# Griffan/FASTQuick

Hardware: AMD Instinct MI355X
Metric: paired_150bp_reads_aligned_per_sec (higher is better)
Workload: dtype u32

## Files before the change

fastquick_amd/csrc/fq_device.hip:

```cpp
#include <hip/hip_runtime.h>
#include <hip/hip_ext.h>

#include <algorithm>
#include <condition_variable>
#include <atomic>
#include <cstdio>
#include <cstdlib>
#include <cstring>
#include <mutex>
#include <string>
#include <unordered_map>
#include <vector>
#include <sys/mman.h>
#include <sys/syscall.h>
#include <unistd.h>

#include "fq_backend.h"

namespace fqdev {

struct Pending { int kid; hipEvent_t a, b; };
struct State {
  int device = 0;
  hipStream_t stream = nullptr;
// ... 368 lines not shown
  uint32_t *cursor;
  const uint32_t *split;
  uint32_t n_work;
  int pref, seg, n_seg;
  __device__ uint64_t operator()(uint32_t n) const {
    const uint32_t sp = split ? *split : n_work;
    const uint32_t blk_start[2] = {0u, sp}, blk_len[2] = {sp, n_work - sp};
    for (int t = 0; t < 2; ++t) {
      const int b = t == 0 ? pref : 1 - pref;
      uint32_t lo, hi;
      fq_seg_range(blk_len[b], seg, n_seg, &lo, &hi);
      const uint32_t len = hi - lo;
      if (len == 0) continue;
      if (__hip_atomic_load(&cursor[b], __ATOMIC_RELAXED, __HIP_MEMORY_SCOPE_AGENT) >= len) continue;
      const uint32_t base = atomicAdd(&cursor[b], n);
      if (base < len) return (uint64_t)(blk_start[b] + lo + base) | (uint64_t)(blk_start[b] + hi) << 32;
    }
    return 0;
  }
};
#define FQ_LANE_FETCH(a) FqQueueFetch2{(a).queue, (a).split, (uint32_t)(a).n_work, (int)((blockIdx.x & 7u) >> 2), (a).seg, (a).n_seg}
__global__ void __launch_bounds__(64) FQ_GAP_OCC k_gap_persist_lds(FqGapArgs a) {
  uint16_t *heads = (uint16_t *)fq_dyn_lds;
  FqGapStoreLds st = {heads + threadIdx.x, 64, (uint32_t *)(heads + 64 * a.o.n_buckets) + threadIdx.x};
  fq_gap_lanes<false>(a, st, FQ_LANE_FETCH(a), (int)(blockIdx.x * 64 + threadIdx.x));
}
__global__ void __launch_bounds__(64) FQ_NOGAP_OCC k_gap_nogap_lds(FqGapArgs a) {
  uint16_t *heads = (uint16_t *)fq_dyn_lds;
  FqGapStoreLds st = {heads + threadIdx.x, 64, (uint32_t *)(heads + 64 * a.o.n_buckets) + threadIdx.x};
  fq_gap_lanes<true>(a, st, FQ_LANE_FETCH(a), (int)(blockIdx.x * 64 + threadIdx.x));
}
__global__ void __launch_bounds__(64) FQ_GAP_OCC k_gap_persist_stock(FqGapArgs a) {
  uint16_t *heads = (uint16_t *)fq_dyn_lds;
  FqGapStoreLds st = {heads + threadIdx.x, 64, (uint32_t *)(heads + 64 * a.o.n_buckets) + threadIdx.x};
  fq_gap_lanes<false, FqOptsStock>(a, st, FQ_LANE_FETCH(a), (int)(blockIdx.x * 64 + threadIdx.x));
}
__global__ void __launch_bounds__(64) FQ_NOGAP_OCC k_gap_nogap_stock(FqGapArgs a) {
  uint16_t *heads = (uint16_t *)fq_dyn_lds;
  FqGapStoreLds st = {heads + threadIdx.x, 64, (uint32_t *)(heads + 64 * a.o.n_buckets) + threadIdx.x};
  fq_gap_lanes<true, FqOptsStock>(a, st, FQ_LANE_FETCH(a), (int)(blockIdx.x * 64 + threadIdx.x));
}
__global__ void __launch_bounds__(64) k_gap_persist(FqGapArgs a) {
  FqGapStoreGlobal st = {nullptr, {}};
  fq_gap_lanes<false>(a, st, FQ_LANE_FETCH(a), (int)(blockIdx.x * 64 + threadIdx.x));
}
__global__ void __launch_bounds__(64) k_gap_coop(FqGapArgs a) {
  __shared__ uint32_t heads[2 * FQ_MAX_BUCKETS];
  fq_gap_coop_wave(a, heads, FqQueueFetch{a.queue, a.n_work}, (int)blockIdx.x);
}
__global__ void __launch_bounds__(256) k_sa(FqSaArgs a) {
  const uint64_t q = (uint64_t)blockIdx.x * blockDim.x + threadIdx.x;
  if (q < a.n_rows) fq_sa_thread(a, q);
}
template <bool PACKED>
__device__ int fq_global_align_wave(const uint8_t *s1, int len1, const uint8_t *s2, int len2, int band, int gap_end,
                                    int *RM, int *RI, int *RD, uint8_t *trace, uint8_t *ops, int *n_ops, int *fi, int *fj);
__device__ __forceinline__ int fq_wave_incl_max(int x, int lane) {
#pragma unroll
  for (int d = 1; d < 64; d <<= 1) { const int y = __shfl_up(x, d, 64); if (lane >= d) x = x > y ? x : y; }
  return x;
}
__device__ void fq_sw_reverse_wave(const uint8_t *ref, const uint8_t *qry, int score_f, int end_i, int end_j, int *H, int *E, int *start_i_out, int *start_j_out, int *score_r_out) {
  const int lane = threadIdx.x;
  const int q = FQ_GAP_O, rr = FQ_GAP_E, qr = q + rr;
  const int kNeg = -(1 << 29);
  for (int i = lane; i <= end_i; i += 64) { H[i] = 0; E[i] = 0; }
  __syncthreads();
  int score_r = fq_sm_maq(ref[end_i - 1], qry[end_j - 1]);
  int start_i = end_i, start_j = end_j;
  if (lane == 0) { H[end_i] = qr + score_r; E[end_i] = 0; }
  __syncthreads();
  int start = end_i - 1, end = end_i - 3;
  if (end <= 0) end = 0;
  bool stop = false;
  for (int j = end_j - 1; j != 0; --j) {
    const int c2 = qry[j - 1];
    const int n = start - end;
    int carry_b = kNeg, carry_m = score_r;
    int d_in = 0, s_in = 0, e_in = 0;
    if (lane < n) { const int i = start - lane; d_in = H[i + 1]; s_in = H[i]; e_in = E[i + 1]; }
    for (int g0 = 0; g0 < n; g0 += 64) {
      const int g = g0 + lane, i = start - g;
      const bool act = g < n;
      int d_nx = 0, s_nx = 0, e_nx = 0;
      if (g + 64 < n) { const int i2 = i - 64; d_nx = H[i2 + 1]; s_nx = H[i2]; e_nx = E[i2 + 1]; }
      int e = e_in - rr > s_in - qr ? e_in - rr : s_in - qr;
      if (e < 0) e = 0;
      int a0 = act ? d_in + fq_sm_maq(ref[i - 1], c2) : 0;
      if (a0 < 0) a0 = 0;
      if (a0 < e) a0 = e;
      const int b = act ? a0 - q + g * rr : kNeg;
      const int bi = fq_wave_incl_max(b, lane);
      int bx = __shfl_up(bi, 1, 64);
      if (lane == 0) bx = kNeg;
      if (bx < carry_b) bx = carry_b;
      const int fpos = bx - g * rr;
      const int h = a0 > fpos ? a0 : fpos;
      const int b_last = __shfl(bi, 63, 64);
      if (carry_b < b_last) carry_b = b_last;
      const int mi = fq_wave_incl_max(act ? h : kNeg, lane);
      int mx = __shfl_up(mi, 1, 64);
      if (lane == 0) mx = kNeg;
      if (mx < carry_m) mx = carry_m;
      const bool improve = act && h > mx;
      const unsigned long long stops = __ballot(improve && h - qr == score_f);
      if (stops) {
        const int ls = __ffsll((long long)stops) - 1;
// ... 51 lines not shown
    for (int d = 32; d >= 1; d >>= 1) nn += __shfl_xor(nn, d, 64);
    if ((float)nn / len >= 0.25f || len - nn < 20) ok = false;
    const int64_t avail = l_pac - T.beg;
    len1 = (int)(avail < (int64_t)T.reglen ? avail : (int64_t)T.reglen);
    if (len1 < 0) len1 = 0;
    for (int k = lane; k < len1; k += 64) ref[k] = (uint8_t)fq_pac_base(a.ix.pac, T.beg + k);
    for (int k = lane; k <= len1 + 1; k += 64) { Hb[k] = 0; Eb[k] = 0; }
  }
  __syncthreads();
  if (!ok) { if (lane == 0) a.out[t] = O; return; }
  const int len2 = len;
  int best_h = 0, best_i = 0, best_j = 0;
  for (int j0 = 0; j0 < len2; j0 += 64) {
    const int j = j0 + lane + 1;
    const bool active = j <= len2;
    const int c2 = active ? qry[j - 1] : 4;
    const int nrows = len2 - j0 < 64 ? len2 - j0 : 64;
    int last_h = 0, f = 0, diag = 0, out_h = 0, out_e = 0;
    const int steps = len1 + nrows - 1;
    for (int st = 1; st <= steps; ++st) {
      int up_h = __shfl_up(out_h, 1, 64), up_e = __shfl_up(out_e, 1, 64);
      const int i = st - lane;
      const bool in = active && i >= 1 && i <= len1;
      if (lane == 0 && in) { up_h = Hb[i]; up_e = Eb[i]; }
      if (in) {
        int e_out;
        const int h = fq_sw_cell(diag, up_h, up_e, fq_sm_maq(ref[i - 1], c2), last_h, f, e_out);
        diag = up_h;
        out_h = h; out_e = e_out;
        if (best_h < h) { best_h = h; best_i = i; best_j = j; }
        if (lane == nrows - 1) { Hb[i] = h; Eb[i] = e_out; }
      }
    }
    __syncthreads();
  }
#pragma unroll
  for (int d = 32; d >= 1; d >>= 1) {
    const int oh = __shfl_xor(best_h, d, 64), oi = __shfl_xor(best_i, d, 64), oj = __shfl_xor(best_j, d, 64);
    if (oh > best_h || (oh == best_h && oh > 0 && oj < best_j)) { best_h = oh; best_i = oi; best_j = oj; }
  }
  if (best_h < 1) { if (lane == 0) a.out[t] = O; return; }
  FqDpScratch S = fq_dp_carve(a.scratch + (size_t)t * a.scratch_stride, RL, QL);
  uint8_t *ops = qry + ((QL + 16) & ~15);
  uint8_t *trace = a.trace_in_lds ? ops + ((RL + QL + 16) & ~15) : S.trace;
  int start_i = 0, start_j = 0, score_r = 0;
  if (a.serial_reverse) {
    if (lane == 0) fq_sw_reverse(ref, qry, best_h, best_i, best_j, Hb, Eb, &start_i, &start_j, &score_r);
    start_i = __shfl(start_i, 0); start_j = __shfl(start_j, 0); score_r = __shfl(score_r, 0);
  } else fq_sw_reverse_wave(ref, qry, best_h, best_i, best_j, Hb, Eb, &start_i, &start_j, &score_r);
  __syncthreads();
  int n_ops = 0, fi = 0, fj = 0, score_g;
  const int jmax = (best_i - start_i > best_j - start_j ? best_i - start_i : best_j - start_j) + 1;
  for (int b = FQ_BAND;; b <<= 1) {
    score_g = fq_global_align_wave<false>(ref + start_i - 1, best_i - start_i + 1, qry + start_j - 1, best_j - start_j + 1, b, -1, rM, rI, rD, trace, ops, &n_ops, &fi, &fj);
    if (score_g == score_r || best_h == score_g) break;
    if (b > jmax) break;
  }
  if (lane == 0) {
    if (!(score_r > score_g && best_h > score_g))
      fq_sw_post(T, ref, qry, len, best_j, start_i, start_j, fi, fj, ops, n_ops, a.cigar + (size_t)t * (size_t)a.cig_cap, a.cig_cap, O);
    a.out[t] = O;
  }
}

__global__ void __launch_bounds__(64) k_refine_lds(FqRefineArgs a) {
  const int t = blockIdx.x * 64 + threadIdx.x;
  int *base = (int *)fq_dyn_lds;
  const int W = a.RL + 1;
  FqRowsPlanar R = {base + threadIdx.x, base + (size_t)W * 64 + threadIdx.x, base + (size_t)2 * W * 64 + threadIdx.x, 64};
  if (t < a.n_task) fq_refine_task(a, t, R);
}
template <bool PACKED>
__device__ __forceinline__ uint8_t fq_trace_get(const uint8_t *trace, int W, int j, int i) {
  if (!PACKED) return trace[(size_t)j * W + i];
  return (uint8_t)((trace[(size_t)j * ((W + 1) >> 1) + (i >> 1)] >> (4 * (i & 1))) & 15);
}
template <bool PACKED>
__device__ int fq_global_align_wave(const uint8_t *s1, int len1, const uint8_t *s2, int len2, int band, int gap_end,
                                    int *RM, int *RI, int *RD, uint8_t *trace, uint8_t *ops, int *n_ops, int *fi, int *fj) {
  const int lane = threadIdx.x;
  if (len1 == 0 || len2 == 0) { *n_ops = 0; return 0; }
  int b1, b2;
  if (len1 > len2) { b1 = len1 - len2 + band; b2 = band; } else { b1 = band; b2 = len2 - len1 + band; }
  if (b1 > len1) b1 = len1;
  if (b2 > len2) b2 = len2;
  const int W = len1 + 1;
  const int end_ext = gap_end >= 0 ? gap_end : FQ_GAP_E;
  if (lane == 0) {
    uint8_t fm;
    int lM = 0, lD = FQ_NEG_INF;
    RM[0] = 0; RI[0] = RD[0] = FQ_NEG_INF;
    for (int i = 1; i < b1; ++i) {
      const int d = fq_pick_gap(lM, lD, end_ext, fm);
      if (PACKED) { uint8_t *b = trace + (i >> 1); *b = (uint8_t)((i & 1) ? ((*b & 15) | ((fm ? 0 : 8) << 4)) : (fm ? 0 : 8)); }
      else trace[i] = (uint8_t)(fm ? 0 : 8);
      RM[i] = RI[i] = FQ_NEG_INF; RD[i] = d;
      lM = FQ_NEG_INF; lD = d;
    }
  }
  __syncthreads();
  const int p1_end = b2 < len2 ? b2 : len2 - 1;
  for (int j0 = 1; j0 <= len2; j0 += 64) {
    const int j = j0 + lane;
    const bool row_on = j <= len2;
    int phase;
    if (j <= p1_end) phase = 1;
    else if (j == p1_end + 1 && j == len2 && b2 != len2 - 1) phase = 5;
    else if (j <= len2 - b2 + 1) phase = 2;
    else if (j < len2) phase = 3;
    else phase = 4;
    const bool p15 = phase == 1 || phase == 5, endD = phase == 5 || phase == 4;
    const int c0 = p15 ? 0 : j - b2;
    const int hi = !row_on ? -1 : p15 ? ((j + b1 <= len1 + 1) ? j + b1 - 1 : len1) : (phase == 2 ? j + b1 - 1 : len1);
    const int c2 = row_on ? s2[j - 1] : 0;
    const bool keeps_row = row_on && (lane == 63 || j == len2);
    uint8_t *tr = trace + (size_t)j * (size_t)(PACKED ? (W + 1) >> 1 : W);
    uint32_t half = 0;
    const int n_rows = len2 - j0 + 1 < 64 ? len2 - j0 + 1 : 64;
    const int t0 = __shfl(c0, 0), t1 = len1 + n_rows - 1;
    int oM = 0, oI = 0, oD = 0;
    FqCell diag, left;
    diag.M = diag.I = diag.D = 0; left = diag;
    for (int t = t0; t <= t1; ++t) {
      const int i = t - lane;
      FqCell up;
      up.M = __shfl_up(oM, 1); up.I = __shfl_up(oI, 1); up.D = __shfl_up(oD, 1);
      if (lane == 0) { const int ii = i < 0 ? 0 : (i > len1 ? len1 : i); up.M = RM[ii]; up.I = RI[ii]; up.D = RD[ii]; }
      if (row_on && i >= c0 && i <= hi) {
        FqCell c;
        uint8_t fm;
        if (i == c0) {
          c.M = c.I = c.D = FQ_NEG_INF;
          uint8_t tb0 = 0;
          if (p15) { c.I = fq_pick_gap(up.M, up.I, end_ext, fm); tb0 = (uint8_t)(fm ? 0 : 4); }
          if (!PACKED) { if (p15) tr[0] = tb0; }
          else if (i & 1) tr[i >> 1] = (uint8_t)(tb0 << 4);
          else { half = tb0; tr[i >> 1] = tb0; }
        } else {
          uint8_t tM, tb;
          c.M = fq_pick_M(diag, fq_sm_maq(s1[i - 1], c2), tM);
          tb = tM;
          if (i != hi) { c.I = fq_pick_gap(up.M, up.I, FQ_GAP_E, fm); tb |= (uint8_t)(fm ? 0 : 4); }
          else if (p15) {
            if (j + b1 - 1 > len1) { c.I = fq_pick_gap(up.M, up.I, end_ext, fm); tb |= (uint8_t)(fm ? 0 : 4); }
            else c.I = FQ_NEG_INF;
          } else if (phase == 2) c.I = FQ_NEG_INF;
          else { c.I = fq_pick_gap(up.M, up.I, end_ext, fm); tb |= (uint8_t)(fm ? 0 : 4); }
          c.D = fq_pick_gap(left.M, left.D, endD ? end_ext : FQ_GAP_E, fm);
          tb |= (uint8_t)(fm ? 0 : 8);
          if (!PACKED) tr[i] = tb;
          else if (i & 1) tr[i >> 1] = (uint8_t)(half | (uint32_t)tb << 4);
          else { half = tb; tr[i >> 1] = tb; }
        }
        diag = up; left = c;
        oM = c.M; oI = c.I; oD = c.D;
        if (keeps_row) { RM[i] = c.M; RI[i] = c.I; RD[i] = c.D; }
      }
    }
    __syncthreads();
  }
  int mx = 0, n = 0, li = 0, lj = 0;
  if (lane == 0) {
    int i = len1, j = len2;
    mx = RM[len1];
    uint8_t tb = fq_trace_get<PACKED>(trace, W, j, i);
    int type = tb & 3, ctype = FQ_OP_M;
    if (RI[len1] > mx) { mx = RI[len1]; type = (tb & 4) ? FQ_OP_I : FQ_OP_M; ctype = FQ_OP_I; }
    if (RD[len1] > mx) { mx = RD[len1]; type = (tb & 8) ? FQ_OP_D : FQ_OP_M; ctype = FQ_OP_D; }
    li = i; lj = j;
    ops[n++] = (uint8_t)ctype;
    do {
      if (ctype == FQ_OP_M) { --i; --j; } else if (ctype == FQ_OP_I) --j; else --i;
      ctype = type;
      tb = fq_trace_get<PACKED>(trace, W, j, i);
      type = type == FQ_OP_M ? (tb & 3) : type == FQ_OP_I ? ((tb & 4) ? FQ_OP_I : FQ_OP_M) : ((tb & 8) ? FQ_OP_D : FQ_OP_M);
      if (i || j) { ops[n++] = (uint8_t)ctype; li = i; lj = j; }
    } while (i || j);
  }
  __syncthreads();
  *n_ops = __shfl(n, 0); *fi = __shfl(li, 0); *fj = __shfl(lj, 0);
  return __shfl(mx, 0);
}
__global__ void __launch_bounds__(64) k_refine_wave(FqRefineArgs a) {
  const int t = blockIdx.x, lane = threadIdx.x;
  const int RL = a.RL, QL = a.QL;
  int *RM = (int *)fq_dyn_lds, *RI = RM + (RL + 1), *RD = RI + (RL + 1);
  uint8_t *ref = (uint8_t *)(RD + (RL + 1));
  uint8_t *qry = ref + ((RL + 16) & ~15);
  uint8_t *ops = qry + ((QL + 16) & ~15);
  uint8_t *trace = ops + ((RL + QL + 16) & ~15);
  const FqRefTask T = a.task[t];
  const int len = a.len_trim[T.read];
  const uint8_t *row = a.seq + (size_t)T.read * (size_t)a.stride;
  const int64_t l_pac = a.ix.l_pac;
  for (int k = lane; k < len; k += 64) qry[k] = (uint8_t)(T.strand ? fq_comp(fq_nt4(row[len - 1 - k])) : fq_nt4(row[k]));
  int64_t pos = (int64_t)T.pos > l_pac ? (int64_t)(int32_t)T.pos : (int64_t)T.pos;
  const int aext = T.ext < 0 ? -T.ext : T.ext, ref_len = len + aext;
  int64_t k0, k1;
  if (T.ext > 0) { k0 = pos; k1 = pos + ref_len < l_pac ? pos + ref_len : l_pac; }
  else { const int64_t x = pos + len; k0 = x - ref_len > 0 ? x - ref_len : 0; k1 = x < l_pac ? x : l_pac; }
  const int l = k1 > k0 ? (int)(k1 - k0) : 0;
  for (int k = lane; k < l; k += 64) ref[k] = (uint8_t)fq_pac_base(a.ix.pac, k0 + k);
  __syncthreads();
  int n_ops = 0, fi, fj;
  fq_global_align_wave<true>(ref, l, qry, len, FQ_BAND, FQ_GAP_END, RM, RI, RD, trace, ops, &n_ops, &fi, &fj);
  if (lane != 0) return;
  uint16_t *cg = a.cigar + (size_t)t * (size_t)a.cig_cap;
  int n = fq_ops_to_cigar(ops, n_ops, cg, a.cig_cap);
  FqRefOut O;
  if (n <= 0) { O.pos = T.pos; O.n_cigar = 0; a.out[t] = O; return; }
  if (T.ext < 0) {
    int d = 0;
    for (int k = 0; k < n; ++k) { const int op = cg[k] >> 14, ln = cg[k] & 0x3fff; if (op == FQ_OP_D) d -= ln; else if (op == FQ_OP_I) d += ln; }
    pos += d;
  }
  if ((cg[0] >> 14) == FQ_OP_D) { pos += cg[0] & 0x3fff; for (int k = 0; k < n - 1; ++k) cg[k] = cg[k + 1]; --n; }
  if ((cg[n - 1] >> 14) == FQ_OP_D) --n;
  if ((cg[n - 1] >> 14) == FQ_OP_I) cg[n - 1] = (uint16_t)(FQ_OP_S << 14 | (cg[n - 1] & 0x3fff));
  if ((cg[0] >> 14) == FQ_OP_I) cg[0] = (uint16_t)(FQ_OP_S << 14 | (cg[0] & 0x3fff));
  O.pos = (uint32_t)pos; O.n_cigar = n;
  a.out[t] = O;
}
__global__ void __launch_bounds__(64) k_refine(FqRefineArgs a) {
  const int t = blockIdx.x * blockDim.x + threadIdx.x;
  if (t < a.n_task) fq_refine_thread(a, t);
}
__global__ void __launch_bounds__(256) k_pack_aln(const FqAln *aln, const uint32_t *n_aln, const uint64_t *off, uint32_t cap, uint32_t n_work, FqAln *packed) {
  const uint32_t w = blockIdx.x * blockDim.x + threadIdx.x;
  if (w >= n_work) return;
  const uint32_t n = n_aln[w];
  const uint64_t o = off[w];
  for (uint32_t j = 0; j < n; ++j) packed[o + j] = aln[(size_t)w * cap + j];
}

__device__ __forceinline__ uint32_t block_excl_scan(uint32_t v, uint32_t *total) {
  __shared__ uint32_t wsum[4];
  const int lane = threadIdx.x & 63, wid = threadIdx.x >> 6;
  uint32_t x = v;
#pragma unroll
  for (int d = 1; d < 64; d <<= 1) {
    const uint32_t y = __shfl_up(x, d, 64);
    if (lane >= d) x += y;
  }
  if (lane == 63) wsum[wid] = x;
  __syncthreads();
  uint32_t base = 0, tot = 0;
#pragma unroll
  for (int k = 0; k < 4; ++k) { if (k < wid) base += wsum[k]; tot += wsum[k]; }
  __syncthreads();
  *total = tot;
  return base + x - v;
}

__global__ void __launch_bounds__(256) k_scan_a(const uint32_t *in, uint32_t n, uint64_t *blk_tot) {
  const uint32_t i = blockIdx.x * 256 + threadIdx.x;
  uint32_t tot;
  (void)block_excl_scan(i < n ? in[i] : 0u, &tot);
  if (threadIdx.x == 0) blk_tot[blockIdx.x] = tot;
}
__global__ void __launch_bounds__(256) k_scan_b(uint64_t *blk_tot, uint32_t nb) {
  __shared__ uint64_t carry;
  if (threadIdx.x == 0) carry = 0;
  __syncthreads();
  for (uint32_t base = 0; base < nb; base += 256) {
    const uint32_t i = base + threadIdx.x;
    const uint64_t v = i < nb ? blk_tot[i] : 0;
    const int lane = threadIdx.x & 63, wid = threadIdx.x >> 6;
    __shared__ uint64_t ws[4];
    uint64_t x = v;
#pragma unroll
    for (int d = 1; d < 64; d <<= 1) {
      const uint64_t y = __shfl_up(x, d, 64);
      if (lane >= d) x += y;
// ... 563 lines not shown
  }
  FQ_HIP(hipGetLastError());
  return 0;
}
int launch_pack_aln(const FqAln *aln, const uint32_t *n_aln, const uint64_t *off, uint32_t cap, uint32_t n_work, FqAln *packed) {
  FQ_PRE();
  if (!n_work) return 0;
  hipLaunchKernelGGL(k_pack_aln, dim3(nblk(n_work, 256)), dim3(256), 0, g_stream, aln, n_aln, off, cap, n_work, packed);
  FQ_HIP(hipGetLastError());
  return 0;
}
int launch_sa(const FqSaArgs &a) {
  FQ_PRE();
  if (!a.n_rows) return 0;
  hipEvent_t e0, e1;
  kernel_events(FQ_K_SA_KERNEL, &e0, &e1);
  hipExtLaunchKernelGGL(k_sa, dim3(nblk(a.n_rows, 256)), dim3(256), 0, g_stream, e0, e1, 0, a);
  FQ_HIP(hipGetLastError());
  return 0;
}
static const size_t kLdsBudget = 150 * 1024;
int launch_sw(const FqSwArgs &a) {
  FQ_PRE();
  if (a.n_task <= 0) return 0;
  size_t lds = (size_t)(2 * (a.RL + 2) + 3 * (a.RL + 1)) * 4 + ((a.RL + 16) & ~15) + ((a.QL + 16) & ~15) + ((a.RL + a.QL + 16) & ~15);
  if (lds > kLdsBudget) { g_err = "SW window too large for LDS (" + std::to_string(a.RL) + " bases)"; return -5; }
  FqSwArgs b = a;
  const size_t trace_bytes = (size_t)(a.RL + 1) * (a.QL + 1) + 16;
  b.trace_in_lds = (lds + trace_bytes <= kLdsBudget && a.n_task <= 256) ? 1 : 0;
  b.serial_reverse = g_cur->tune.sw_serial_reverse;
  if (b.trace_in_lds) lds += trace_bytes;
  hipEvent_t e0, e1;
  kernel_events(FQ_K_SW_KERNEL, &e0, &e1);
  hipExtLaunchKernelGGL(k_sw_wave, dim3((unsigned)a.n_task), dim3(64), lds, g_stream, e0, e1, 0, b);
  FQ_HIP(hipGetLastError());
  return 0;
}
__global__ void __launch_bounds__(64) k_sw_thread(FqSwArgs a) {
  const int t = blockIdx.x * blockDim.x + threadIdx.x;
  if (t < a.n_task) fq_sw_thread(a, t);
}
int launch_sw_serial(const FqSwArgs &a) {
  FQ_PRE();
  if (a.n_task <= 0) return 0;
  hipEvent_t e0, e1;
  kernel_events(FQ_K_SW_KERNEL, &e0, &e1);
  hipExtLaunchKernelGGL(k_sw_thread, dim3(nblk((uint64_t)a.n_task, 64)), dim3(64), 0, g_stream, e0, e1, 0, a);
  FQ_HIP(hipGetLastError());
  return 0;
}
int launch_refine(const FqRefineArgs &a) {
  FQ_PRE();
  if (a.n_task <= 0) return 0;
  const size_t wave_lds = (size_t)3 * (a.RL + 1) * 4 + ((a.RL + 16) & ~15) + ((a.QL + 16) & ~15) + ((a.RL + a.QL + 16) & ~15) + (size_t)((a.RL + 2) >> 1) * (a.QL + 1) + 16;
  const bool no_wave = g_cur->tune.refine_lanes != 0;
  hipEvent_t e0, e1;
  kernel_events(FQ_K_REFINE_KERNEL, &e0, &e1);
  if (wave_lds <= 64 * 1024 && !no_wave) {
    hipExtLaunchKernelGGL(k_refine_wave, dim3((unsigned)a.n_task), dim3(64), wave_lds, g_stream, e0, e1, 0, a);
    FQ_HIP(hipGetLastError());
    return 0;
  }
  const size_t lds = (size_t)3 * (a.RL + 1) * 64 * 4;
  if (lds <= kLdsBudget) {
    hipExtLaunchKernelGGL(k_refine_lds, dim3(nblk((uint64_t)a.n_task, 64)), dim3(64), lds, g_stream, e0, e1, 0, a);
  } else {
    hipExtLaunchKernelGGL(k_refine, dim3(nblk((uint64_t)a.n_task, 64)), dim3(64), 0, g_stream, e0, e1, 0, a);
  }
  FQ_HIP(hipGetLastError());
  return 0;
}

#define FQ_REC_KERNEL(name, body)                                                    \
  __global__ void __launch_bounds__(256) name(FqRecArgs a, int n) {                  \
    const int i = blockIdx.x * blockDim.x + threadIdx.x;                             \
    if (i < n) body(a, i);                                                           \
  }
FQ_REC_KERNEL(k_rec_init, fq_rec_init_thread)
FQ_REC_KERNEL(k_rec_nocc, fq_rec_nocc_thread)
FQ_REC_KERNEL(k_enum_plan, fq_enum_plan_thread)
FQ_REC_KERNEL(k_enum_fill, fq_enum_fill_thread)
FQ_REC_KERNEL(k_main_hit, fq_main_hit_thread)
FQ_REC_KERNEL(k_compact_idx, fq_compact_thread)
FQ_REC_KERNEL(k_pair_rec, fq_pair_rec_thread)
FQ_REC_KERNEL(k_pair_gather, fq_pair_gather_thread)
FQ_REC_KERNEL(k_pair_scatter, fq_pair_scatter_thread)
FQ_REC_KERNEL(k_xa_count, fq_xa_count_thread)
FQ_REC_KERNEL(k_xa_fill, fq_xa_fill_thread)
FQ_REC_KERNEL(k_sw_plan, fq_sw_plan_thread)
FQ_REC_KERNEL(k_sw_fill, fq_sw_fill_thread)
FQ_REC_KERNEL(k_rec_gather, fq_rec_gather_thread)
FQ_REC_KERNEL(k_rec_scatter, fq_rec_scatter_thread)
FQ_REC_KERNEL(k_ref_count, fq_ref_count_thread)
FQ_REC_KERNEL(k_ref_fill, fq_ref_fill_thread)
FQ_REC_KERNEL(k_ref_apply, fq_ref_apply_thread)
FQ_REC_KERNEL(k_md_rec, fq_md_rec_thread)
FQ_REC_KERNEL(k_md_mask, fq_md_mask_piece)
FQ_REC_KERNEL(k_flat_count, fq_flat_count_thread)
FQ_REC_KERNEL(k_flat_fill, fq_flat_fill_thread)
int launch_rec(int op, const FqRecArgs &a, int64_t n) {
  FQ_PRE();
  if (n <= 0) return 0;
  if (n > 0x7fffffff) { g_err = "record stage: more than 2^31 items"; return -5; }
  typedef void (*Kern)(FqRecArgs, int);
  static const Kern kerns[FQ_ROP_COUNT] = {k_rec_init, k_rec_nocc, k_enum_plan, k_enum_fill, k_main_hit, k_compact_idx, k_pair_rec, k_pair_gather, k_pair_scatter,
                                           k_xa_count, k_xa_fill, k_sw_plan, k_sw_fill, k_rec_gather, k_rec_scatter, k_ref_count, k_ref_fill, k_ref_apply,
                                           k_md_rec, k_md_mask, k_flat_count, k_flat_fill};
// ... 172 lines not shown
```

fastquick_amd/csrc/fq_kernels.h:

```cpp
#pragma once
#include "fq_common.h"

#define FQ_LAMBDA_INLINE __attribute__((always_inline))
#if defined(__HIP_DEVICE_COMPILE__)
#define FQ_POPC64(x) __popcll(x)
#define FQ_POPC32(x) __popc(x)
#define FQ_CTZ32(x) (__ffs((int)(x)) - 1)
#define FQ_C_STRIPE_OFF ((size_t)(blockIdx.x & (FQ_C_STRIPES - 1)) * FQ_C_STRIDE)
#define FQ_ATOMIC_ADD64(p, v) atomicAdd((unsigned long long *)(p) + FQ_C_STRIPE_OFF, (unsigned long long)(v))
#define FQ_ATOMIC_MAX64(p, v) atomicMax((unsigned long long *)(p) + FQ_C_STRIPE_OFF, (unsigned long long)(v))
#define FQ_LOAD_RELAXED(p) __hip_atomic_load((p), __ATOMIC_RELAXED, __HIP_MEMORY_SCOPE_AGENT)
#define FQ_ATOMIC_MAX32(p, v) do { const int fq_v_ = (int)(v); if (fq_v_ > FQ_LOAD_RELAXED((const int *)(p))) atomicMax((int *)(p), fq_v_); } while (0)
#define FQ_WAVE_COUNT(p, pred)                                                                                      \
  do {                                                                                                              \
    const unsigned long long m_ = __ballot((pred) ? 1 : 0);                                                         \
    if ((pred) && __lane_id() == (unsigned)(__ffsll((long long)m_) - 1)) atomicAdd((unsigned long long *)(p) + FQ_C_STRIPE_OFF, (unsigned long long)__popcll(m_)); \
  } while (0)
#else
#define FQ_WAVE_COUNT(p, pred) do { if (pred) *(p) += 1; } while (0)
#define FQ_LOAD_RELAXED(p) (*(p))
#define FQ_ATOMIC_MAX32(p, v) (*(p) = *(p) > (int32_t)(v) ? *(p) : (int32_t)(v))
#define FQ_ATOMIC_MAX64(p, v) (*(p) = *(p) > (uint64_t)(v) ? *(p) : (uint64_t)(v))
#define FQ_POPC64(x) __builtin_popcountll(x)
#define FQ_POPC32(x) __builtin_popcount(x)
// ... 1836 lines not shown
      diag = R.get(j - b2);
      left.M = left.I = left.D = FQ_NEG_INF;
      R.set(j - b2, left);
    }
    for (int i = lo; i <= hi; ++i) {
      const FqCell up = R.get(i);
      FqCell c;
      uint8_t tM, tb;
      c.M = fq_pick_M(diag, fq_sm_maq(s1[i - 1], c2), tM);
      tb = tM;
      if (i != hi) { c.I = fq_pick_gap(up.M, up.I, FQ_GAP_E, fm); tb |= (uint8_t)(fm ? 0 : 4); }
      else if (phase == 1 || phase == 5) {
        if (j + b1 - 1 > len1) { c.I = fq_pick_gap(up.M, up.I, end_ext, fm); tb |= (uint8_t)(fm ? 0 : 4); }
        else c.I = FQ_NEG_INF;
      } else if (phase == 2) c.I = FQ_NEG_INF;
      else { c.I = fq_pick_gap(up.M, up.I, end_ext, fm); tb |= (uint8_t)(fm ? 0 : 4); }
      c.D = fq_pick_gap(left.M, left.D, endD ? end_ext : FQ_GAP_E, fm);
      tb |= (uint8_t)(fm ? 0 : 8);
      tr[i] = tb;
      R.set(i, c);
      diag = up;
      left = c;
    }
  }
  const FqCell last = R.get(len1);
  int i = len1, j = len2, mx = last.M;
  uint8_t tb = trace[(size_t)j * W + i];
  int type = tb & 3, ctype = FQ_OP_M;
  if (last.I > mx) { mx = last.I; type = (tb & 4) ? FQ_OP_I : FQ_OP_M; ctype = FQ_OP_I; }
  if (last.D > mx) { mx = last.D; type = (tb & 8) ? FQ_OP_D : FQ_OP_M; ctype = FQ_OP_D; }
  int n = 0, li = i, lj = j;
  ops[n++] = (uint8_t)ctype;
  do {
    if (ctype == FQ_OP_M) { --i; --j; } else if (ctype == FQ_OP_I) --j; else --i;
    ctype = type;
    tb = trace[(size_t)j * W + i];
    type = type == FQ_OP_M ? (tb & 3) : type == FQ_OP_I ? ((tb & 4) ? FQ_OP_I : FQ_OP_M) : ((tb & 8) ? FQ_OP_D : FQ_OP_M);
    if (i || j) { ops[n++] = (uint8_t)ctype; li = i; lj = j; }
  } while (i || j);
  *n_ops = n;
  *fi = li; *fj = lj;
  return mx;
}

FQ_HD int fq_ops_to_cigar(const uint8_t *ops, int n_ops, uint16_t *cg, int cap) {
  int n = 0;
  for (int t = n_ops - 1; t >= 0; --t) {
    if (n && (cg[n - 1] >> 14) == ops[t]) ++cg[n - 1];
    else { if (n >= cap) return -1; cg[n++] = (uint16_t)(ops[t] << 14 | 1); }
  }
  return n;
}

struct FqDpScratch {
  uint8_t *ref, *qry, *ops, *trace;
  int *H, *E;
  FqCell *rows;
};
FQ_HD size_t fq_dp_scratch_bytes(int RL, int QL) {
  size_t b = 0;
  b += ((size_t)RL + 16) & ~(size_t)15;
  b += ((size_t)QL + 16) & ~(size_t)15;
  b += ((size_t)RL + QL + 16) & ~(size_t)15;
  b += 2 * ((((size_t)RL + 2) * sizeof(int) + 15) & ~(size_t)15);
  b += ((size_t)RL + 1) * sizeof(FqCell) + 16;
  b += ((size_t)RL + 1) * ((size_t)QL + 1) + 16;
  return (b + 63) & ~(size_t)63;
}
FQ_HD FqDpScratch fq_dp_carve(uint8_t *base, int RL, int QL) {
  FqDpScratch s;
  uint8_t *p = base;
  s.ref = p; p += ((size_t)RL + 16) & ~(size_t)15;
  s.qry = p; p += ((size_t)QL + 16) & ~(size_t)15;
  s.ops = p; p += ((size_t)RL + QL + 16) & ~(size_t)15;
  s.H = (int *)p; p += (((size_t)RL + 2) * sizeof(int) + 15) & ~(size_t)15;
  s.E = (int *)p; p += (((size_t)RL + 2) * sizeof(int) + 15) & ~(size_t)15;
  s.rows = (FqCell *)p; p += ((size_t)RL + 1) * sizeof(FqCell) + 16;
  p = (uint8_t *)(((uintptr_t)p + 15) & ~(uintptr_t)15);
  s.trace = p;
  return s;
}

struct FqSwArgs {
  FqDevIndex ix;
  const uint8_t *seq;
  int32_t stride;
  const int32_t *len_trim;
  const FqSwTask *task;
  int32_t n_task;
  FqSwOut *out;
  uint16_t *cigar;
  int32_t cig_cap;
  uint8_t *scratch;
  size_t scratch_stride;
  int32_t RL, QL;
  int32_t trace_in_lds;
  int32_t serial_reverse;
};

FQ_HD int fq_sw_cell(int diag, int up, int e_up, int sc, int &last_h, int &f, int &e_out) {
  const int q = FQ_GAP_O, r = FQ_GAP_E, qr = q + r;
  int h = diag + sc;
  if (h < 0) h = 0;
  if (last_h > 0) { f = f > last_h - q ? f - r : last_h - qr; if (h < f) h = f; }
  if (up >= qr + 1) { const int e = e_up > up - q ? e_up - r : up - qr; if (h < e) h = e; e_out = e; }
  else e_out = 0;
// ... 167 lines not shown
    fq_sw_finish(T, S.ref, len1, S.qry, len, score_f, end_i, end_j, S.H, S.E, R, S.trace, S.ops, A.cigar + (size_t)t * (size_t)A.cig_cap, A.cig_cap, O);
  }
  A.out[t] = O;
}

struct FqRefineArgs {
  FqDevIndex ix;
  const uint8_t *seq;
  int32_t stride;
  const int32_t *len_trim;
  const FqRefTask *task;
  int32_t n_task;
  FqRefOut *out;
  uint16_t *cigar;
  int32_t cig_cap;
  uint8_t *scratch;
  size_t scratch_stride;
  int32_t RL, QL;
};
template <class Rows>
FQ_HD void fq_refine_task(const FqRefineArgs &A, int t, const Rows &R) {
  const FqRefTask T = A.task[t];
  const int len = A.len_trim[T.read];
  const uint8_t *row = A.seq + (size_t)T.read * (size_t)A.stride;
  const int64_t l_pac = A.ix.l_pac;
  FqDpScratch S = fq_dp_carve(A.scratch + (size_t)t * A.scratch_stride, A.RL, A.QL);
  for (int k = 0; k < len; ++k) S.qry[k] = (uint8_t)(T.strand ? fq_comp(fq_nt4(row[len - 1 - k])) : fq_nt4(row[k]));
  int64_t pos = (int64_t)T.pos > l_pac ? (int64_t)(int32_t)T.pos : (int64_t)T.pos;
  const int aext = T.ext < 0 ? -T.ext : T.ext, ref_len = len + aext;
  int l = 0;
  if (T.ext > 0) { for (int64_t k = pos; k < pos + ref_len && k < l_pac; ++k) S.ref[l++] = (uint8_t)fq_pac_base(A.ix.pac, k); }
  else {
    const int64_t x = pos + len;
    for (int64_t k = x - ref_len > 0 ? x - ref_len : 0; k < x && k < l_pac; ++k) S.ref[l++] = (uint8_t)fq_pac_base(A.ix.pac, k);
  }
  int n_ops = 0, fi, fj;
  fq_global_align(S.ref, l, S.qry, len, FQ_BAND, FQ_GAP_END, R, S.trace, S.ops, &n_ops, &fi, &fj);
  uint16_t *cg = A.cigar + (size_t)t * (size_t)A.cig_cap;
  int n = fq_ops_to_cigar(S.ops, n_ops, cg, A.cig_cap);
  FqRefOut O;
  if (n <= 0) { O.pos = T.pos; O.n_cigar = 0; A.out[t] = O; return; }
  if (T.ext < 0) {
    int d = 0;
    for (int k = 0; k < n; ++k) { const int op = cg[k] >> 14, ln = cg[k] & 0x3fff; if (op == FQ_OP_D) d -= ln; else if (op == FQ_OP_I) d += ln; }
    pos += d;
  }
  if ((cg[0] >> 14) == FQ_OP_D) { pos += cg[0] & 0x3fff; for (int k = 0; k < n - 1; ++k) cg[k] = cg[k + 1]; --n; }
  if ((cg[n - 1] >> 14) == FQ_OP_D) --n;
  if ((cg[n - 1] >> 14) == FQ_OP_I) cg[n - 1] = (uint16_t)(FQ_OP_S << 14 | (cg[n - 1] & 0x3fff));
  if ((cg[0] >> 14) == FQ_OP_I) cg[0] = (uint16_t)(FQ_OP_S << 14 | (cg[0] & 0x3fff));
  O.pos = (uint32_t)pos; O.n_cigar = n;
  A.out[t] = O;
}
FQ_HD void fq_refine_thread(const FqRefineArgs &A, int t) {
  FqDpScratch S = fq_dp_carve(A.scratch + (size_t)t * A.scratch_stride, A.RL, A.QL);
  FqRowsArr R = {S.rows};
  fq_refine_task(A, t, R);
}

FQ_HD int fq_put_int(char *dst, int at, int cap, int v) {
  char tmp[12]; int n = 0;
  if (v == 0) tmp[n++] = '0';
  while (v > 0) { tmp[n++] = (char)('0' + v % 10); v /= 10; }
  while (n > 0) { if (at < cap) dst[at] = tmp[n - 1]; ++at; --n; }
  return at;
}
FQ_HD void fq_md_core(const FqDevIndex &ix, const uint8_t *row, const FqMdTask &T, const uint16_t *cigar_arena, char *dst, int cap, int *at_out, int *nm_out) {
  const int64_t l_pac = ix.l_pac;
  const int slen = T.len;
  uint32_t x = T.pos, y = 0;
  int u = 0, nm = 0, at = 0;
  if (T.n_cigar) {
    const uint16_t *cg = cigar_arena + T.cigar_off;
    for (int k = 0; k < T.n_cigar; ++k) {
      const int op = cg[k] >> 14, l = cg[k] & 0x3fff;
      if (op == FQ_OP_M) {
        for (int z = 0; z < l && (int64_t)(uint32_t)(x + z) < l_pac; ++z) {
          const int c = fq_pac_base(ix.pac, (int64_t)(uint32_t)(x + z));
          const int yy = (int)y + z;
          const int sc = T.strand ? fq_comp(fq_nt4(row[slen - 1 - yy])) : fq_nt4(row[yy]);
          if (sc > 3 || c != sc) { at = fq_put_int(dst, at, cap, u); if (at < cap) dst[at] = "ACGTN"[c]; ++at; ++nm; u = 0; }
          else ++u;
        }
        x += l; y += l;
      } else if (op == FQ_OP_I || op == FQ_OP_S) { y += l; if (op == FQ_OP_I) nm += l; }
      else {
        at = fq_put_int(dst, at, cap, u);
        if (at < cap) dst[at] = '^';
        ++at;
        for (int z = 0; z < l && (int64_t)(uint32_t)(x + z) < l_pac; ++z) { if (at < cap) dst[at] = "ACGT"[fq_pac_base(ix.pac, (int64_t)(uint32_t)(x + z))]; ++at; }
        u = 0; x += l; nm += l;
      }
    }
  } else {
    int z = 0;
    for (; z + 8 <= slen; z += 8) {
      uint64_t rb;
      uint32_t pb;
      memcpy(&rb, T.strand ? row + (slen - 8 - z) : row + z, 8);
      const uint32_t k0 = x + (uint32_t)z;
      memcpy(&pb, ix.pac + (k0 >> 2), 4);
#pragma unroll
      for (int j = 0; j < 8; ++j) {
        const uint32_t kk = k0 + (uint32_t)j;
        const int c = (int)((pb >> (8 * ((kk >> 2) - (k0 >> 2)))) >> ((~kk & 3u) << 1)) & 3;
        const int ch = (int)(rb >> (8 * (T.strand ? 7 - j : j))) & 0xff;
// ... 92 lines not shown
```

Before: 774.1 million.

## Rewrite wave refine as anti-diagonal banded DP with ballot-driven traceback

Replaces the row-block wave global alignment in the refine kernel with a banded anti-diagonal formulation. Each of 64 lanes owns two band cells, neighbours are exchanged via shuffles, and traceback is packed into a compact band-indexed LDS buffer. Traceback is done wave-parallel: lanes probe 64 steps ahead and a ballot finds where the run breaks, emitting CIGAR runs directly. Tasks whose band does not fit in 128 cells fall back to the scalar thread path. The intent is to cut per-cell work, LDS footprint and serial traceback cost, at the price of more complex indexing and possible divergence in the fallback path.

```diff
diff --git a/fastquick_amd/csrc/fq_device.hip b/fastquick_amd/csrc/fq_device.hip
--- a/fastquick_amd/csrc/fq_device.hip
+++ b/fastquick_amd/csrc/fq_device.hip
@@ -444,7 +444,6 @@
   const uint64_t q = (uint64_t)blockIdx.x * blockDim.x + threadIdx.x;
   if (q < a.n_rows) fq_sa_thread(a, q);
 }
-template <bool PACKED>
 __device__ int fq_global_align_wave(const uint8_t *s1, int len1, const uint8_t *s2, int len2, int band, int gap_end,
                                     int *RM, int *RI, int *RD, uint8_t *trace, uint8_t *ops, int *n_ops, int *fi, int *fj);
 __device__ __forceinline__ int fq_wave_incl_max(int x, int lane) {
@@ -602,7 +601,7 @@
   int n_ops = 0, fi = 0, fj = 0, score_g;
   const int jmax = (best_i - start_i > best_j - start_j ? best_i - start_i : best_j - start_j) + 1;
   for (int b = FQ_BAND;; b <<= 1) {
-    score_g = fq_global_align_wave<false>(ref + start_i - 1, best_i - start_i + 1, qry + start_j - 1, best_j - start_j + 1, b, -1, rM, rI, rD, trace, ops, &n_ops, &fi, &fj);
+    score_g = fq_global_align_wave(ref + start_i - 1, best_i - start_i + 1, qry + start_j - 1, best_j - start_j + 1, b, -1, rM, rI, rD, trace, ops, &n_ops, &fi, &fj);
     if (score_g == score_r || best_h == score_g) break;
     if (b > jmax) break;
   }
@@ -620,12 +619,6 @@
   FqRowsPlanar R = {base + threadIdx.x, base + (size_t)W * 64 + threadIdx.x, base + (size_t)2 * W * 64 + threadIdx.x, 64};
   if (t < a.n_task) fq_refine_task(a, t, R);
 }
-template <bool PACKED>
-__device__ __forceinline__ uint8_t fq_trace_get(const uint8_t *trace, int W, int j, int i) {
-  if (!PACKED) return trace[(size_t)j * W + i];
-  return (uint8_t)((trace[(size_t)j * ((W + 1) >> 1) + (i >> 1)] >> (4 * (i & 1))) & 15);
-}
-template <bool PACKED>
 __device__ int fq_global_align_wave(const uint8_t *s1, int len1, const uint8_t *s2, int len2, int band, int gap_end,
                                     int *RM, int *RI, int *RD, uint8_t *trace, uint8_t *ops, int *n_ops, int *fi, int *fj) {
   const int lane = threadIdx.x;
@@ -642,8 +635,7 @@
     RM[0] = 0; RI[0] = RD[0] = FQ_NEG_INF;
     for (int i = 1; i < b1; ++i) {
       const int d = fq_pick_gap(lM, lD, end_ext, fm);
-      if (PACKED) { uint8_t *b = trace + (i >> 1); *b = (uint8_t)((i & 1) ? ((*b & 15) | ((fm ? 0 : 8) << 4)) : (fm ? 0 : 8)); }
-      else trace[i] = (uint8_t)(fm ? 0 : 8);
+      trace[i] = (uint8_t)(fm ? 0 : 8);
       RM[i] = RI[i] = FQ_NEG_INF; RD[i] = d;
       lM = FQ_NEG_INF; lD = d;
     }
@@ -664,8 +656,7 @@
     const int hi = !row_on ? -1 : p15 ? ((j + b1 <= len1 + 1) ? j + b1 - 1 : len1) : (phase == 2 ? j + b1 - 1 : len1);
     const int c2 = row_on ? s2[j - 1] : 0;
     const bool keeps_row = row_on && (lane == 63 || j == len2);
-    uint8_t *tr = trace + (size_t)j * (size_t)(PACKED ? (W + 1) >> 1 : W);
-    uint32_t half = 0;
+    uint8_t *tr = trace + (size_t)j * (size_t)W;
     const int n_rows = len2 - j0 + 1 < 64 ? len2 - j0 + 1 : 64;
     const int t0 = __shfl(c0, 0), t1 = len1 + n_rows - 1;
     int oM = 0, oI = 0, oD = 0;
@@ -681,11 +672,7 @@
         uint8_t fm;
         if (i == c0) {
           c.M = c.I = c.D = FQ_NEG_INF;
-          uint8_t tb0 = 0;
-          if (p15) { c.I = fq_pick_gap(up.M, up.I, end_ext, fm); tb0 = (uint8_t)(fm ? 0 : 4); }
-          if (!PACKED) { if (p15) tr[0] = tb0; }
-          else if (i & 1) tr[i >> 1] = (uint8_t)(tb0 << 4);
-          else { half = tb0; tr[i >> 1] = tb0; }
+          if (p15) { c.I = fq_pick_gap(up.M, up.I, end_ext, fm); tr[0] = (uint8_t)(fm ? 0 : 4); }
         } else {
           uint8_t tM, tb;
           c.M = fq_pick_M(diag, fq_sm_maq(s1[i - 1], c2), tM);
@@ -698,9 +685,7 @@
           else { c.I = fq_pick_gap(up.M, up.I, end_ext, fm); tb |= (uint8_t)(fm ? 0 : 4); }
           c.D = fq_pick_gap(left.M, left.D, endD ? end_ext : FQ_GAP_E, fm);
           tb |= (uint8_t)(fm ? 0 : 8);
-          if (!PACKED) tr[i] = tb;
-          else if (i & 1) tr[i >> 1] = (uint8_t)(half | (uint32_t)tb << 4);
-          else { half = tb; tr[i >> 1] = tb; }
+          tr[i] = tb;
         }
         diag = up; left = c;
         oM = c.M; oI = c.I; oD = c.D;
@@ -713,7 +698,7 @@
   if (lane == 0) {
     int i = len1, j = len2;
     mx = RM[len1];
-    uint8_t tb = fq_trace_get<PACKED>(trace, W, j, i);
+    uint8_t tb = trace[(size_t)j * W + i];
     int type = tb & 3, ctype = FQ_OP_M;
     if (RI[len1] > mx) { mx = RI[len1]; type = (tb & 4) ? FQ_OP_I : FQ_OP_M; ctype = FQ_OP_I; }
     if (RD[len1] > mx) { mx = RD[len1]; type = (tb & 8) ? FQ_OP_D : FQ_OP_M; ctype = FQ_OP_D; }
@@ -722,7 +707,7 @@
     do {
       if (ctype == FQ_OP_M) { --i; --j; } else if (ctype == FQ_OP_I) --j; else --i;
       ctype = type;
-      tb = fq_trace_get<PACKED>(trace, W, j, i);
+      tb = trace[(size_t)j * W + i];
       type = type == FQ_OP_M ? (tb & 3) : type == FQ_OP_I ? ((tb & 4) ? FQ_OP_I : FQ_OP_M) : ((tb & 8) ? FQ_OP_D : FQ_OP_M);
       if (i || j) { ops[n++] = (uint8_t)ctype; li = i; lj = j; }
     } while (i || j);
@@ -731,44 +716,68 @@
   *n_ops = __shfl(n, 0); *fi = __shfl(li, 0); *fj = __shfl(lj, 0);
   return __shfl(mx, 0);
 }
+#define FQ_WAVE_UP1(x) __shfl_up((x), 1, 64)
+#define FQ_WAVE_DOWN1(x) __shfl_down((x), 1, 64)
+__device__ int fq_refine_band_wave(const FqBandGeom &G, const uint8_t *s1, const uint8_t *s2, uint8_t *trace, uint16_t *runs, int cap) {
+  const int lane = threadIdx.x;
+  FqBandLane L;
+  L.A.M = L.A.I = L.A.D = 0; L.B = L.A;
+  const int r1 = fq_band_last_iter(G);
+  for (int r = -1; r <= r1; ++r) {
+    const int lM = FQ_WAVE_UP1(L.B.M), lD = FQ_WAVE_UP1(L.B.D);
+    const uint32_t ta = fq_band_half_a(G, s1, s2, lane, r, L, lM, lD);
+    const int uM = FQ_WAVE_DOWN1(L.A.M), uI = FQ_WAVE_DOWN1(L.A.I);
+    const uint32_t tb = fq_band_half_b(G, s1, s2, lane, r, L, uM, uI);
+    fq_band_trace_put(trace, fq_band_row(G, lane, r), lane, ta, tb);
+  }
+  const FqCell mine = fq_band_end_cell(G, L);
+  const int el = fq_band_end_lane(G);
+  FqCell last;
+  last.M = (int)FQ_READLANE32(mine.M, el); last.I = (int)FQ_READLANE32(mine.I, el); last.D = (int)FQ_READLANE32(mine.D, el);
+  __syncthreads();
+  int i = G.len1, j = G.len2, t = fq_band_first_state(last), n = 0;
+  while ((i | j) > 0) {
+    const uint32_t p = fq_band_probe(G, trace, i, j, t, lane);
+    const uint64_t stops = FQ_BALLOT(p & 4);
+    const int cnt = stops ? FQ_CTZ64(stops) + 1 : 64;
+    if (lane == 0) n = fq_band_run_push(runs, n, cap, t, cnt);
+    n = (int)FQ_READLANE32(n, 0);
+    if (t != FQ_OP_I) i -= cnt;
+    if (t != FQ_OP_D) j -= cnt;
+    t = (int)FQ_READLANE32(p, cnt - 1) & 3;
+  }
+  __syncthreads();
+  return n;
+}
 __global__ void __launch_bounds__(64) k_refine_wave(FqRefineArgs a) {
   const int t = blockIdx.x, lane = threadIdx.x;
   const int RL = a.RL, QL = a.QL;
-  int *RM = (int *)fq_dyn_lds, *RI = RM + (RL + 1), *RD = RI + (RL + 1);
-  uint8_t *ref = (uint8_t *)(RD + (RL + 1));
+  uint8_t *ref = (uint8_t *)fq_dyn_lds;
   uint8_t *qry = ref + ((RL + 16) & ~15);
-  uint8_t *ops = qry + ((QL + 16) & ~15);
-  uint8_t *trace = ops + ((RL + QL + 16) & ~15);
+  uint16_t *runs = (uint16_t *)(qry + ((QL + 16) & ~15));
+  uint8_t *trace = (uint8_t *)(runs + ((a.cig_cap + 7) & ~7));
   const FqRefTask T = a.task[t];
   const int len = a.len_trim[T.read];
   const uint8_t *row = a.seq + (size_t)T.read * (size_t)a.stride;
   const int64_t l_pac = a.ix.l_pac;
-  for (int k = lane; k < len; k += 64) qry[k] = (uint8_t)(T.strand ? fq_comp(fq_nt4(row[len - 1 - k])) : fq_nt4(row[k]));
-  int64_t pos = (int64_t)T.pos > l_pac ? (int64_t)(int32_t)T.pos : (int64_t)T.pos;
+  const int64_t pos = (int64_t)T.pos > l_pac ? (int64_t)(int32_t)T.pos : (int64_t)T.pos;
   const int aext = T.ext < 0 ? -T.ext : T.ext, ref_len = len + aext;
   int64_t k0, k1;
   if (T.ext > 0) { k0 = pos; k1 = pos + ref_len < l_pac ? pos + ref_len : l_pac; }
   else { const int64_t x = pos + len; k0 = x - ref_len > 0 ? x - ref_len : 0; k1 = x < l_pac ? x : l_pac; }
   const int l = k1 > k0 ? (int)(k1 - k0) : 0;
+  const FqBandGeom G = fq_band_geom(l, len, FQ_BAND, FQ_GAP_END);
+  if (l > 0 && len > 0 && !fq_band_fits(G)) {
+    if (lane == 0) fq_refine_thread(a, t);
+    return;
+  }
+  for (int k = lane; k < len; k += 64) qry[k] = (uint8_t)(T.strand ? fq_comp(fq_nt4(row[len - 1 - k])) : fq_nt4(row[k]));
   for (int k = lane; k < l; k += 64) ref[k] = (uint8_t)fq_pac_base(a.ix.pac, k0 + k);
   __syncthreads();
-  int n_ops = 0, fi, fj;
-  fq_global_align_wave<true>(ref, l, qry, len, FQ_BAND, FQ_GAP_END, RM, RI, RD, trace, ops, &n_ops, &fi, &fj);
+  const int n = (l > 0 && len > 0) ? fq_refine_band_wave(G, ref, qry, trace, runs, a.cig_cap) : 0;
   if (lane != 0) return;
-  uint16_t *cg = a.cigar + (size_t)t * (size_t)a.cig_cap;
-  int n = fq_ops_to_cigar(ops, n_ops, cg, a.cig_cap);
   FqRefOut O;
-  if (n <= 0) { O.pos = T.pos; O.n_cigar = 0; a.out[t] = O; return; }
-  if (T.ext < 0) {
-    int d = 0;
-    for (int k = 0; k < n; ++k) { const int op = cg[k] >> 14, ln = cg[k] & 0x3fff; if (op == FQ_OP_D) d -= ln; else if (op == FQ_OP_I) d += ln; }
-    pos += d;
-  }
-  if ((cg[0] >> 14) == FQ_OP_D) { pos += cg[0] & 0x3fff; for (int k = 0; k < n - 1; ++k) cg[k] = cg[k + 1]; --n; }
-  if ((cg[n - 1] >> 14) == FQ_OP_D) --n;
-  if ((cg[n - 1] >> 14) == FQ_OP_I) cg[n - 1] = (uint16_t)(FQ_OP_S << 14 | (cg[n - 1] & 0x3fff));
-  if ((cg[0] >> 14) == FQ_OP_I) cg[0] = (uint16_t)(FQ_OP_S << 14 | (cg[0] & 0x3fff));
-  O.pos = (uint32_t)pos; O.n_cigar = n;
+  fq_refine_finish(runs, n, T.ext, pos, T.pos, a.cigar + (size_t)t * (size_t)a.cig_cap, a.cig_cap, O);
   a.out[t] = O;
 }
 __global__ void __launch_bounds__(64) k_refine(FqRefineArgs a) {
@@ -1438,7 +1447,7 @@
 int launch_refine(const FqRefineArgs &a) {
   FQ_PRE();
   if (a.n_task <= 0) return 0;
-  const size_t wave_lds = (size_t)3 * (a.RL + 1) * 4 + ((a.RL + 16) & ~15) + ((a.QL + 16) & ~15) + ((a.RL + a.QL + 16) & ~15) + (size_t)((a.RL + 2) >> 1) * (a.QL + 1) + 16;
+  const size_t wave_lds = (size_t)((a.RL + 16) & ~15) + ((a.QL + 16) & ~15) + (size_t)((a.cig_cap + 7) & ~7) * 2 + (size_t)fq_band_trace_bytes(a.QL) + 16;
   const bool no_wave = g_cur->tune.refine_lanes != 0;
   hipEvent_t e0, e1;
   kernel_events(FQ_K_REFINE_KERNEL, &e0, &e1);
diff --git a/fastquick_amd/csrc/fq_kernels.h b/fastquick_amd/csrc/fq_kernels.h
--- a/fastquick_amd/csrc/fq_kernels.h
+++ b/fastquick_amd/csrc/fq_kernels.h
@@ -1912,6 +1912,110 @@
   return n;
 }
 
+#define FQ_BAND_LANES 64
+struct FqBandGeom {
+  int len1, len2, b1, b2, end_ext;
+  int p1_end, j5, p2_last;
+  int h;
+};
+FQ_HD FqBandGeom fq_band_geom(int len1, int len2, int band, int gap_end) {
+  FqBandGeom G;
+  int b1, b2;
+  if (len1 > len2) { b1 = len1 - len2 + band; b2 = band; } else { b1 = band; b2 = len2 - len1 + band; }
+  if (b1 > len1) b1 = len1;
+  if (b2 > len2) b2 = len2;
+  G.len1 = len1; G.len2 = len2; G.b1 = b1; G.b2 = b2;
+  G.end_ext = gap_end >= 0 ? gap_end : FQ_GAP_E;
+  G.p1_end = b2 < len2 ? b2 : len2 - 1;
+  G.j5 = (G.p1_end + 1 == len2 && b2 != len2 - 1) ? len2 : -1;
+  G.p2_last = len2 - b2 + 1;
+  G.h = (b2 + 1) >> 1;
+  return G;
+}
+FQ_HD bool fq_band_fits(const FqBandGeom &G) { return G.len1 > 0 && G.len2 > 0 && G.b1 + G.b2 <= 2 * FQ_BAND_LANES; }
+FQ_HD int fq_band_last_iter(const FqBandGeom &G) { return G.len2 + ((G.len1 - G.len2 + G.b2) >> 1) - G.h; }
+FQ_HD int fq_band_trace_bytes(int len2) { return FQ_BAND_LANES * (len2 + 1); }
+FQ_HD bool fq_band_cell(const FqBandGeom &G, const uint8_t *s1, const uint8_t *s2, int i, int j, const FqCell &diag, int upM, int upI, int leftM, int leftD,
+                        FqCell &c, uint32_t &tb) {
+  uint8_t fm;
+  if (j < 0 || j > G.len2 || i < 0 || i > G.len1) return false;
+  if (j == 0) {
+    if (i >= G.b1) return false;
+    c.M = i ? FQ_NEG_INF : 0; c.I = c.D = FQ_NEG_INF; tb = 0;
+    if (i) { c.D = fq_pick_gap(leftM, leftD, G.end_ext, fm); tb = fm ? 0 : 8; }
+    return true;
+  }
+  const int phase = j <= G.p1_end ? 1 : j == G.j5 ? 5 : j <= G.p2_last ? 2 : j < G.len2 ? 3 : 4;
+  const bool p15 = phase == 1 || phase == 5, endD = phase == 5 || phase == 4;
+  const int c0 = p15 ? 0 : j - G.b2;
+  const int hi = p15 ? ((j + G.b1 <= G.len1 + 1) ? j + G.b1 - 1 : G.len1) : (phase == 2 ? j + G.b1 - 1 : G.len1);
+  if (i < c0 || i > hi) return false;
+  if (i == c0) {
+    c.M = c.I = c.D = FQ_NEG_INF; tb = 0;
+    if (p15) { c.I = fq_pick_gap(upM, upI, G.end_ext, fm); tb = fm ? 0 : 4; }
+    return true;
+  }
+  uint8_t tM;
+  c.M = fq_pick_M(diag, fq_sm_maq(s1[i - 1], s2[j - 1]), tM);
+  tb = tM;
+  if (i != hi) { c.I = fq_pick_gap(upM, upI, FQ_GAP_E, fm); tb |= fm ? 0 : 4; }
+  else if (p15) {
+    if (j + G.b1 - 1 > G.len1) { c.I = fq_pick_gap(upM, upI, G.end_ext, fm); tb |= fm ? 0 : 4; }
+    else c.I = FQ_NEG_INF;
+  } else if (phase == 2) c.I = FQ_NEG_INF;
+  else { c.I = fq_pick_gap(upM, upI, G.end_ext, fm); tb |= fm ? 0 : 4; }
+  c.D = fq_pick_gap(leftM, leftD, endD ? G.end_ext : FQ_GAP_E, fm);
+  tb |= fm ? 0 : 8;
+  return true;
+}
+struct FqBandLane { FqCell A, B; };
+FQ_HD int fq_band_row(const FqBandGeom &G, int k, int r) { return r - k + G.h; }
+FQ_HD uint32_t fq_band_half_a(const FqBandGeom &G, const uint8_t *s1, const uint8_t *s2, int k, int r, FqBandLane &L, int lM, int lD) {
+  const int j = fq_band_row(G, k, r), i = j + 2 * k - G.b2;
+  FqCell c;
+  uint32_t tb;
+  if (!fq_band_cell(G, s1, s2, i, j, L.A, L.B.M, L.B.I, lM, lD, c, tb)) return 0;
+  L.A = c;
+  return tb | 16;
+}
+FQ_HD uint32_t fq_band_half_b(const FqBandGeom &G, const uint8_t *s1, const uint8_t *s2, int k, int r, FqBandLane &L, int uM, int uI) {
+  const int j = fq_band_row(G, k, r), i = j + 2 * k - G.b2 + 1;
+  FqCell c;
+  uint32_t tb;
+  if (!fq_band_cell(G, s1, s2, i, j, L.B, uM, uI, L.A.M, L.A.D, c, tb)) return 0;
+  L.B = c;
+  return tb | 16;
+}
+FQ_HD void fq_band_trace_put(uint8_t *trace, int j, int k, uint32_t ta, uint32_t tb) {
+  if ((ta | tb) & 16) trace[j * FQ_BAND_LANES + k] = (uint8_t)((ta & 15) | (tb & 15) << 4);
+}
+FQ_HD uint32_t fq_band_trace_get(const FqBandGeom &G, const uint8_t *trace, int i, int j) {
+  const int e = (i - j + G.b2) & (2 * FQ_BAND_LANES - 1);
+  return (uint32_t)(trace[j * FQ_BAND_LANES + (e >> 1)] >> (4 * (e & 1))) & 15;
+}
+FQ_HD int fq_band_end_lane(const FqBandGeom &G) { return (G.len1 - G.len2 + G.b2) >> 1; }
+FQ_HD FqCell fq_band_end_cell(const FqBandGeom &G, const FqBandLane &L) { return ((G.len1 - G.len2 + G.b2) & 1) ? L.B : L.A; }
+FQ_HD int fq_trace_pred(int t, uint32_t tb) { return t == FQ_OP_M ? (int)(tb & 3) : t == FQ_OP_I ? ((tb & 4) ? FQ_OP_I : FQ_OP_M) : ((tb & 8) ? FQ_OP_D : FQ_OP_M); }
+FQ_HD int fq_band_first_state(const FqCell &last) {
+  int mx = last.M, t = FQ_OP_M;
+  if (last.I > mx) { mx = last.I; t = FQ_OP_I; }
+  if (last.D > mx) t = FQ_OP_D;
+  return t;
+}
+FQ_HD uint32_t fq_band_probe(const FqBandGeom &G, const uint8_t *trace, int i, int j, int t, int l) {
+  const int di = t != FQ_OP_I, dj = t != FQ_OP_D;
+  const int ci = i - l * di, cj = j - l * dj;
+  if (ci < 0 || cj < 0) return 4u | (uint32_t)t;
+  const int ni = ci - di, nj = cj - dj;
+  const int pred = fq_trace_pred(t, fq_band_trace_get(G, trace, ci, cj));
+  return ((pred != t || ni < 0 || nj < 0 || (ni | nj) == 0) ? 4u : 0u) | (uint32_t)pred;
+}
+FQ_HD int fq_band_run_push(uint16_t *runs, int n, int cap, int t, int cnt) {
+  if (n && n <= cap && (runs[n - 1] >> 14) == t) { runs[n - 1] = (uint16_t)(runs[n - 1] + cnt); return n; }
+  if (n < cap) runs[n] = (uint16_t)(t << 14 | cnt);
+  return n + 1;
+}
+
 struct FqDpScratch {
   uint8_t *ref, *qry, *ops, *trace;
   int *H, *E;
@@ -2185,6 +2289,24 @@
   O.pos = (uint32_t)pos; O.n_cigar = n;
   A.out[t] = O;
 }
+FQ_HD void fq_refine_finish(const uint16_t *runs, int n, int ext, int64_t pos, uint32_t task_pos, uint16_t *cg, int cap, FqRefOut &O) {
+  if (n <= 0 || n > cap) { O.pos = task_pos; O.n_cigar = 0; return; }
+  if (ext < 0) {
+    int d = 0;
+    for (int k = 0; k < n; ++k) { const int op = runs[k] >> 14, ln = runs[k] & 0x3fff; if (op == FQ_OP_D) d -= ln; else if (op == FQ_OP_I) d += ln; }
+    pos += d;
+  }
+  int lo = 0, hi = n;
+  if ((runs[n - 1] >> 14) == FQ_OP_D) { pos += runs[n - 1] & 0x3fff; lo = 1; }
+  if (hi > lo && (runs[n - hi] >> 14) == FQ_OP_D) --hi;
+  const int m = hi - lo;
+  for (int k = 0; k < m; ++k) {
+    uint16_t g = runs[n - 1 - (k + lo)];
+    if ((k == 0 || k == m - 1) && (g >> 14) == FQ_OP_I) g = (uint16_t)(FQ_OP_S << 14 | (g & 0x3fff));
+    cg[k] = g;
+  }
+  O.pos = (uint32_t)pos; O.n_cigar = m;
+}
 FQ_HD void fq_refine_thread(const FqRefineArgs &A, int t) {
   FqDpScratch S = fq_dp_carve(A.scratch + (size_t)t * A.scratch_stride, A.RL, A.QL);
   FqRowsArr R = {S.rows};
```

New measurement: 776.8 million (median of 3 runs). No clear change (+0.3%).
